# chongkuiqi/S2ANet

Measured on AMD Instinct MI355X. Metric: 1024x1024 DOTA chips/sec (R-50-FPN S2ANet inference), higher is better.
Workload: dtype f16; 1 GPU; BASELINE configs[2]: full R-50-FPN S2ANet inference, batch 8 of 1024x1024 synthetic uint8 chips per GPU; 3 independent batches in flight on 3 HIP streams; global_batch=8, num_classes=15, weights=seeded random init of the reference architecture; odm_cls bias calibrated, nms_candidate_cap=160000, nms_candidates_dropped=0, distinct_input_batches=3, fam_cls_branch=True, hip_graph=False, batches_in_flight=3, parallelism=dp1 (one process per GPU)

## Files before the change

include/s2anet_hip.h:

```cpp
#ifndef S2ANET_HIP_H_
#define S2ANET_HIP_H_

#include <stddef.h>
#include <stdint.h>

#ifdef __cplusplus
extern "C" {
#endif

#define S2A_OK 0
#define S2A_EINVAL (-1)
#define S2A_EWORKSPACE (-2)
#define S2A_EHIP (-3)
#define S2A_ENOTIMPL (-4)

#define S2A_DTYPE_F32 0
#define S2A_DTYPE_F16 1
#define S2A_DTYPE_F64 2

#define S2A_LAYOUT_NCHW 0
#define S2A_LAYOUT_NHWC 1

typedef void* s2a_stream_t;

// ... 217 lines not shown
int s2a_deform_conv_backward_input_f32(const float* input, const float* offset, const float* grad_output, const float* weight,
                                       float* grad_input, float* grad_offset, int64_t batch, int64_t channels,
                                       int64_t height, int64_t width, int64_t out_channels, void* workspace,
                                       size_t workspace_bytes, s2a_stream_t stream);

size_t s2a_deform_conv_backward_weight_workspace_bytes(int64_t batch, int64_t channels, int64_t height, int64_t width,
                                                       int64_t out_channels);
int s2a_deform_conv_backward_weight_f16(const void* input, const void* offset, const void* grad_output,
                                        float* grad_weight_f32, int64_t batch, int64_t channels, int64_t height,
                                        int64_t width, int64_t out_channels, void* workspace, size_t workspace_bytes,
                                        s2a_stream_t stream);

size_t s2a_deform_conv_backward_weight_f32_workspace_bytes(int64_t batch, int64_t channels, int64_t height, int64_t width,
                                                           int64_t out_channels);
int s2a_deform_conv_backward_weight_f32(const float* input, const float* offset, const float* grad_output,
                                        float* grad_weight, float scale, int64_t batch, int64_t channels, int64_t height,
                                        int64_t width, int64_t out_channels, void* workspace, size_t workspace_bytes,
                                        s2a_stream_t stream);

size_t s2a_deform_conv_backward_workspace_bytes(int dtype, int64_t batch, int64_t channels, int64_t height, int64_t width,
                                                int64_t out_channels);
int s2a_deform_conv_backward(int dtype, const void* input, const void* offset, const void* grad_output, const void* weight,
                             float* grad_input_f32, void* grad_offset, float* grad_weight_f32, float scale, int64_t batch,
                             int64_t channels, int64_t height, int64_t width, int64_t out_channels, void* workspace,
                             size_t workspace_bytes, s2a_stream_t stream);
int s2a_deform_conv_backward_typed(int dtype, const void* input, const void* offset, const void* grad_output,
                                   const void* weight, void* grad_input, void* grad_offset, float* grad_weight_f32,
                                   float scale, int64_t batch, int64_t channels, int64_t height, int64_t width,
                                   int64_t out_channels, void* workspace, size_t workspace_bytes, s2a_stream_t stream);

int s2a_conv3x3_tail1x1_f16(const void* x, const void* weight_frag, const void* bias, const void* tail_weight_frag,
                            const void* tail_bias, const void* residual, void* out, const void* chain_weight_frag,
                            const void* chain_bias, void* chain_out, int64_t chain_channels, int64_t batch, int64_t channels,
                            int64_t mid_channels, int64_t out_channels, int64_t height, int64_t width,
                            s2a_stream_t stream);

int s2a_conv1x1_chain_f16(const void* x, const void* weight_frag, const void* bias, const void* residual, void* out,
                          const void* chain_weight_frag, const void* chain_bias, void* chain_out, int64_t chain_channels,
                          int64_t batch, int64_t channels, int64_t out_channels, int64_t height, int64_t width,
                          s2a_stream_t stream);

int s2a_conv1x1_add_up2_f16(const void* x, const void* weight_frag, const void* bias, const void* coarse,
                            void* out, int64_t batch, int64_t channels, int64_t height, int64_t width,
                            int64_t out_channels, s2a_stream_t stream);

int64_t s2a_pyramid_pixels(const s2a_pyramid* pyr, int64_t batch);
int s2a_conv3x3_pyramid_f16(const void* x, const void* weight_frag, const void* bias, const void* residual,
                            void* out, int64_t batch, int64_t channels, int64_t out_channels, int relu,
                            const s2a_pyramid* pyr, s2a_stream_t stream);
int s2a_conv3x3_head_pyramid_f16(const void* x, const void* weight_frag, const void* bias, void* out,
                                 const void* head_weight_frag, const void* head_bias, void* head_out,
                                 int64_t batch, int64_t channels, int64_t out_channels, int relu,
                                 const s2a_pyramid* pyr, s2a_stream_t stream);
int s2a_orconv_pool_pyramid_f16(const void* x, const void* weight_frag, const void* bias, void* out, void* pooled,
                                int64_t batch, int64_t channels, int64_t out_channels, const s2a_pyramid* pyr,
                                s2a_stream_t stream);
int64_t s2a_conv_wino_packed_elems(int64_t out_channels, int64_t channels);
int s2a_conv_wino_pack_weight_f16(const void* weight, int64_t out_channels, int64_t channels, void* packed,
                                  s2a_stream_t stream);
int s2a_conv3x3_wino_pyramid_f16(const void* x, const void* weight_wino, const void* bias, void* out, void* pooled,
                                 int64_t batch, int64_t channels, int64_t out_channels, int relu,
                                 const s2a_pyramid* pyr, s2a_stream_t stream);
int s2a_align_conv_pyramid_f16(const void* x, const float* anchors, const void* weight_packed, void* out,
                               int64_t batch, int64_t channels, int64_t out_channels, int relu,
                               const s2a_pyramid* pyr, s2a_stream_t stream);
int s2a_fam_refine_anchors_pyramid(const void* pred, int64_t row_stride, int64_t batch, const s2a_pyramid* pyr,
                                   float anchor_scale, float* refined, s2a_stream_t stream);

int64_t s2a_stem_packed_elems(void);
int s2a_stem_pack_weight_f16(const void* weight, void* packed, s2a_stream_t stream);
int s2a_stem_u8_f16(const void* image_u8, const void* weight_packed, const void* bias, void* out,
                    int64_t batch, int64_t height, int64_t width, float divisor, s2a_stream_t stream);

#define S2A_LOSS_MAX_LEVELS 8

typedef struct s2a_loss_map {
  const void* cls;
  const void* bbox;
  const float* anchors;
  float* grad_cls;
  float* grad_bbox;
  int64_t anchor_batch_stride;
  int32_t height, width;
  int32_t cls_dtype, bbox_dtype;
  float fpn_balance;
  int32_t reserved;
} s2a_loss_map;

typedef struct s2a_loss_params {
  int32_t batch, num_classes, n_levels, reserved;
  float fl_gamma, fl_alpha, smooth_l1_beta, reg_balance, odm_balance;
  s2a_loss_map map[2][S2A_LOSS_MAX_LEVELS];
} s2a_loss_params;

size_t s2a_s2anet_loss_workspace_bytes(int64_t batch, int64_t anchors_per_image);
int s2a_s2anet_loss_forward(const s2a_loss_params* params, const int64_t* assign_ids, const float* targets,
                            const int64_t* target_offsets, float* loss, float* items, float* norm, void* workspace,
                            size_t workspace_bytes, s2a_stream_t stream);

typedef struct s2a_loss_grad_map {
  const float* src;
  void* dst;
  int64_t numel;
  int32_t dtype;
  int32_t norm_index;
} s2a_loss_grad_map;
// ... 50 lines not shown
```

s2anet_amd/_lib.py:

```python
import ctypes
import os
import subprocess

import torch

_HERE = os.path.dirname(os.path.abspath(__file__))
LIB_PATH = os.environ.get("S2A_LIB_PATH") or os.path.join(_HERE, "libs2anet_hip.so")

OK, EINVAL, EWORKSPACE, EHIP, ENOTIMPL = 0, -1, -2, -3, -4
DTYPE_F32, DTYPE_F16, DTYPE_F64 = 0, 1, 2
LAYOUT_NCHW, LAYOUT_NHWC = 0, 1

c_i64, c_int, c_f32, c_sz, c_vp = (ctypes.c_int64, ctypes.c_int, ctypes.c_float, ctypes.c_size_t,
                                   ctypes.c_void_p)


class DcnParams(ctypes.Structure):
    _fields_ = [("batch", c_i64), ("channels", c_i64), ("height", c_i64), ("width", c_i64),
                ("out_channels", c_i64),
                ("kW", c_int), ("kH", c_int), ("dW", c_int), ("dH", c_int), ("padW", c_int),
                ("padH", c_int), ("dilationW", c_int), ("dilationH", c_int), ("group", c_int),
                ("deformable_group", c_int), ("dtype", c_int), ("offset_dtype", c_int),
                ("layout", c_int), ("relu", c_int)]

# ... 98 lines not shown
    "s2a_s2anet_loss_workspace_bytes": (c_sz, [c_i64, c_i64]),
    "s2a_s2anet_loss_forward": (c_int, [ctypes.POINTER(LossParams), c_vp, c_vp, c_vp, c_vp, c_vp, c_vp, c_vp, c_sz, c_vp]),
    "s2a_s2anet_loss_backward": (c_int, [ctypes.POINTER(LossGradMap), c_int, c_vp, c_vp, c_vp]),
    "s2a_deform_conv_workspace_bytes": (c_sz, [ctypes.POINTER(DcnParams)]),
    "s2a_deform_conv_forward": (c_int, [c_vp, c_vp, c_vp, c_vp, ctypes.POINTER(DcnParams), c_vp,
                                        c_sz, c_vp]),
    "s2a_align_offsets": (c_int, [c_vp, c_i64, c_i64, c_i64, c_f32, c_int, c_vp, c_vp]),
    "s2a_align_conv_workspace_bytes": (c_sz, [ctypes.POINTER(AlignParams)]),
    "s2a_align_conv_forward": (c_int, [c_vp, c_vp, c_vp, c_vp, ctypes.POINTER(AlignParams), c_vp,
                                       c_sz, c_vp]),
    "s2a_dcn_packed_elems": (c_i64, [c_i64, c_i64, c_int]),
    "s2a_nms_small_stats": (c_int, [ctypes.POINTER(ctypes.c_int64), ctypes.POINTER(ctypes.c_int64)]),
    "s2a_dcn_pack_weight": (c_int, [c_vp, c_i64, c_i64, c_int, c_vp, c_vp]),
    "s2a_bias_act_nhwc": (c_int, [c_vp, c_vp, c_vp, c_i64, c_i64, c_int, c_int, c_vp]),
    "s2a_bias_act_nhwc_to": (c_int, [c_vp, c_vp, c_vp, c_vp, c_i64, c_i64, c_int, c_int, c_vp]),
    "s2a_conv_pack_weight_f16": (c_int, [c_vp, c_i64, c_i64, c_int, c_vp, c_vp]),
    "s2a_conv_nhwc_f16": (c_int, [c_vp, c_vp, c_vp, c_vp, c_vp, c_i64, c_i64, c_i64, c_i64, c_i64, c_int, c_int,
                                  c_int, c_vp]),
    "s2a_conv_pack_weight_train": (c_int, [c_vp, c_int, c_i64, c_i64, c_int, c_vp, c_vp, c_vp]),
    "s2a_conv_backward_prep_f16_workspace_bytes": (c_sz, [c_i64, c_i64]),
    "s2a_conv_backward_prep_f16": (c_int, [c_vp, c_vp, c_vp, c_vp, c_int, c_i64, c_i64, c_vp, c_sz, c_vp]),
    "s2a_conv_backward_weight_f16_workspace_bytes": (c_sz, [c_i64, c_i64, c_i64, c_i64, c_i64, c_int]),
    "s2a_conv_backward_weight_f16": (c_int, [c_vp, c_vp, c_vp, c_int, c_i64, c_i64, c_i64, c_i64, c_i64, c_int, c_vp, c_sz,
                                             c_vp]),
    "s2a_debug_read_stamps": (c_int, [c_vp, c_i64]),
    "s2a_build_flags": (c_int, []),
    "s2a_deform_conv_backward_input_workspace_bytes": (c_sz, [c_i64, c_i64, c_i64, c_i64, c_i64]),
    "s2a_deform_conv_backward_weight_workspace_bytes": (c_sz, [c_i64, c_i64, c_i64, c_i64, c_i64]),
    "s2a_deform_conv_backward_workspace_bytes": (c_sz, [c_int, c_i64, c_i64, c_i64, c_i64, c_i64]),
    "s2a_deform_conv_backward": (c_int, [c_int, c_vp, c_vp, c_vp, c_vp, c_vp, c_vp, c_vp, c_f32, c_i64, c_i64, c_i64, c_i64,
                                         c_i64, c_vp, c_sz, c_vp]),
    "s2a_deform_conv_backward_typed": (c_int, [c_int, c_vp, c_vp, c_vp, c_vp, c_vp, c_vp, c_vp, c_f32, c_i64, c_i64, c_i64, c_i64,
                                               c_i64, c_vp, c_sz, c_vp]),
    "s2a_deform_conv_backward_input_f32_workspace_bytes": (c_sz, [c_i64, c_i64, c_i64, c_i64, c_i64]),
    "s2a_deform_conv_backward_weight_f32_workspace_bytes": (c_sz, [c_i64, c_i64, c_i64, c_i64, c_i64]),
    "s2a_deform_conv_backward_weight_f32": (c_int, [c_vp, c_vp, c_vp, c_vp, c_f32, c_i64, c_i64, c_i64, c_i64, c_i64,
                                                    c_vp, c_sz, c_vp]),
    "s2a_deform_conv_backward_input_f32": (c_int, [c_vp, c_vp, c_vp, c_vp, c_vp, c_vp, c_i64, c_i64, c_i64, c_i64, c_i64,
                                                   c_vp, c_sz, c_vp]),
    "s2a_deform_conv_backward_weight_f16": (c_int, [c_vp, c_vp, c_vp, c_vp, c_i64, c_i64, c_i64, c_i64, c_i64, c_vp, c_sz, c_vp]),
    "s2a_deform_conv_backward_input_f16": (c_int, [c_vp, c_vp, c_vp, c_vp, c_vp, c_vp, c_i64, c_i64, c_i64, c_i64, c_i64,
                                           c_vp, c_sz, c_vp]),
    "s2a_deformable_im2col": (c_int, [c_vp, c_vp, c_vp, ctypes.POINTER(DcnParams), c_vp]),
    "s2a_deformable_col2im": (c_int, [c_vp, c_vp, c_vp, ctypes.POINTER(DcnParams), c_vp]),
    "s2a_deformable_col2im_coord": (c_int, [c_vp, c_vp, c_vp, c_vp, ctypes.POINTER(DcnParams), c_vp]),
    "s2a_conv3x3_tail1x1_f16": (c_int, [c_vp] * 10 + [c_i64] * 7 + [c_vp]),
    "s2a_conv1x1_chain_f16": (c_int, [c_vp] * 8 + [c_i64] * 6 + [c_vp]),
    "s2a_conv1x1_add_up2_f16": (c_int, [c_vp, c_vp, c_vp, c_vp, c_vp, c_i64, c_i64, c_i64, c_i64, c_i64, c_vp]),
    "s2a_pyramid_pixels": (c_i64, [ctypes.POINTER(Pyramid), c_i64]),
    "s2a_conv3x3_pyramid_f16": (c_int, [c_vp, c_vp, c_vp, c_vp, c_vp, c_i64, c_i64, c_i64, c_int,
                                        ctypes.POINTER(Pyramid), c_vp]),
    "s2a_conv3x3_head_pyramid_f16": (c_int, [c_vp, c_vp, c_vp, c_vp, c_vp, c_vp, c_vp, c_i64, c_i64, c_i64, c_int,
                                             ctypes.POINTER(Pyramid), c_vp]),
    "s2a_orconv_pool_pyramid_f16": (c_int, [c_vp, c_vp, c_vp, c_vp, c_vp, c_i64, c_i64, c_i64, ctypes.POINTER(Pyramid), c_vp]),
    "s2a_conv_wino_packed_elems": (c_i64, [c_i64, c_i64]),
    "s2a_conv_wino_pack_weight_f16": (c_int, [c_vp, c_i64, c_i64, c_vp, c_vp]),
    "s2a_conv3x3_wino_pyramid_f16": (c_int, [c_vp, c_vp, c_vp, c_vp, c_vp, c_i64, c_i64, c_i64, c_int,
                                             ctypes.POINTER(Pyramid), c_vp]),
    "s2a_align_conv_pyramid_f16": (c_int, [c_vp, c_vp, c_vp, c_vp, c_i64, c_i64, c_i64, c_int,
                                           ctypes.POINTER(Pyramid), c_vp]),
    "s2a_fam_refine_anchors_pyramid": (c_int, [c_vp, c_i64, c_i64, ctypes.POINTER(Pyramid), c_f32, c_vp, c_vp]),
    "s2a_stem_packed_elems": (c_i64, []),
    "s2a_stem_pack_weight_f16": (c_int, [c_vp, c_vp, c_vp]),
    "s2a_stem_u8_f16": (c_int, [c_vp, c_vp, c_vp, c_vp, c_i64, c_i64, c_i64, c_f32, c_vp]),
    "s2a_pyramid_candidates_count": (c_i64, [ctypes.POINTER(Pyramid), c_i64]),
    "s2a_pyramid_candidates": (c_int, [c_vp, c_vp, c_vp, c_i64, ctypes.POINTER(Pyramid), c_int, c_i64, c_f32, c_vp, c_vp, c_vp, c_vp]),
    "s2a_rbox_to_poly": (c_int, [c_vp, c_i64, c_i64, c_vp, c_vp]),
    "s2a_scene_gather_u8": (c_int, [c_vp, c_i64, c_i64, c_vp, c_i64, ctypes.c_int32, c_vp, c_vp]),
    "s2a_scene_merge_workspace_bytes": (c_sz, [c_i64, c_i64]),
    "s2a_scene_merge": (c_int, [c_vp, c_vp, c_vp, c_vp, c_vp, c_i64, c_i64, ctypes.c_int32, ctypes.c_double, c_i64,
                                c_vp, c_vp, c_vp, c_vp, c_vp, c_vp, c_vp, c_sz, c_vp]),
    "s2a_eval_task1_workspace_bytes": (c_sz, [c_i64, c_i64, ctypes.c_int32, ctypes.c_int32]),
    "s2a_eval_task1": (c_int, [c_vp, c_vp, c_vp, c_vp, c_i64, c_vp, c_vp, c_vp, c_vp, c_i64, ctypes.c_int32, ctypes.c_int32,
                               ctypes.c_double, c_int, c_int, ctypes.POINTER(ctypes.c_double)] + [c_vp] * 9 +
                       [ctypes.POINTER(EvalCurves), c_vp, c_sz, c_vp]),
    "s2a_train_update_workspace_bytes": (c_sz, [c_i64]),
    "s2a_train_update": (c_int, [ctypes.POINTER(TrainUpdateArgs), c_vp, c_sz, c_vp]),
    "s2a_delta2bbox_rotated": (c_int, [c_vp, c_vp, c_i64, c_f32, c_vp, c_vp]),
    "s2a_fam_refine_anchors": (c_int, [c_vp, c_i64, c_i64, c_i64, c_f32, c_f32, c_int, c_int,
                                       c_vp, c_vp]),
}


def build(force=False):
    csrc = os.path.join(_HERE, "csrc")
    if force:
        subprocess.check_call(["make", "-C", csrc, "-s", "clean"])
    subprocess.check_call(["make", "-C", csrc, "-s", "-j4"])
    return LIB_PATH


_lib = None


def lib():
    global _lib
    if _lib is None:
        if not os.path.exists(LIB_PATH):
            raise RuntimeError(
                f"{LIB_PATH} is missing: build it with `python -c 'import __graft_entry__ as g; "
                f"g.build()'` or `make -C s2anet_amd/csrc` — s2anet_amd has no CPU fallback")
        L = ctypes.CDLL(LIB_PATH)
        for name, (res, args) in SYMBOLS.items():
            fn = getattr(L, name)
            fn.restype, fn.argtypes = res, args
        flags = L.s2a_build_flags()
# ... 52 lines not shown
```

s2anet_amd/csrc/conv_ops.hip:

```cpp
#include <hip/hip_fp16.h>
#include <hip/hip_runtime.h>

#include <algorithm>
#include <cstdlib>
#include <type_traits>

#include "common.hpp"
#include "mfma_common.hpp"

namespace s2a {
namespace {

__global__ void k_pack_weight_frag(const _Float16* __restrict__ w, int O, int C, _Float16* __restrict__ wp,
                                   int taps = 9) {
  int64_t e = (int64_t)blockIdx.x * blockDim.x + threadIdx.x;
  int64_t total = (int64_t)O * C * taps;
  if (e >= total) return;
  const int G = O / 64;
  int j = (int)(e & 7);
  int lane = (int)((e >> 3) & 63);
  int kk = (int)((e >> 9) & 3);
  int mt = (int)((e >> 11) & 1);
  int64_t r = e >> 12;
  int g = (int)(r % G);
// ... 816 lines not shown
#pragma unroll
      for (int c4 = 0; c4 < 4; c4++)
#pragma unroll
        for (int kk = 0; kk < 4; kk++)
#pragma unroll
          for (int j = 0; j < 2; j++) {
            const V bf = *reinterpret_cast<const V*>(s_st + (32 * j + (lane & 31)) * kStRowB + (c4 * 64 + kk * 16 + (lane >> 5) * 8) * 2);
            c2[j] = __builtin_amdgcn_mfma_f32_32x32x16_f16(aw[c4 * 4 + kk], bf, c2[j], 0, 0, 0);
          }
    }
  }
  __syncthreads();
  constexpr int rowb = O3 * 2 + 16;
  if constexpr (C16) {
#pragma unroll
    for (int n = 0; n < NG3; n++)
#pragma unroll
      for (int a = 0; a < 4; a++) {
        const int och = (wave + 4 * n) * 64 + 16 * a + 4 * kg16;
        const h4e bq = *reinterpret_cast<const h4e*>(chain_b + och);
#pragma unroll
        for (int b = 0; b < 4; b++) {
          h2e lo = {(_Float16)(cacc[n][a][b][0] + (float)bq[0]), (_Float16)(cacc[n][a][b][1] + (float)bq[1])};
          h2e hi = {(_Float16)(cacc[n][a][b][2] + (float)bq[2]), (_Float16)(cacc[n][a][b][3] + (float)bq[3])};
          lo = __builtin_elementwise_max(lo, h2e{(_Float16)0.f, (_Float16)0.f});
          hi = __builtin_elementwise_max(hi, h2e{(_Float16)0.f, (_Float16)0.f});
          *reinterpret_cast<h4e*>(smem + (16 * b + pix16) * rowb + och * 2) = h4e{lo[0], lo[1], hi[0], hi[1]};
        }
      }
  } else {
#pragma unroll
    for (int j = 0; j < 2; j++)
#pragma unroll
      for (int rq = 0; rq < 4; rq++) {
        const int och = wave * 32 + 8 * rq + 4 * (lane >> 5);
        const h4e bq = *reinterpret_cast<const h4e*>(chain_b + och);
        h2e lo = {(_Float16)(c2[j][rq * 4] + (float)bq[0]), (_Float16)(c2[j][rq * 4 + 1] + (float)bq[1])};
        h2e hi = {(_Float16)(c2[j][rq * 4 + 2] + (float)bq[2]), (_Float16)(c2[j][rq * 4 + 3] + (float)bq[3])};
        lo = __builtin_elementwise_max(lo, h2e{(_Float16)0.f, (_Float16)0.f});
        hi = __builtin_elementwise_max(hi, h2e{(_Float16)0.f, (_Float16)0.f});
        *reinterpret_cast<h4e*>(smem + (32 * j + (lane & 31)) * rowb + och * 2) = h4e{lo[0], lo[1], hi[0], hi[1]};
      }
  }
  __syncthreads();
  constexpr int vpr = O3 / 8;
#pragma unroll
  for (int i = 0; i < kPos * vpr / 256; i++) {
    const int idx = tid + 256 * i, pos = idx / vpr, col = idx % vpr;
    if (g0 + pos < Ntot)
      *reinterpret_cast<V*>(chain_out + (g0 + pos) * O3 + col * 8) = *reinterpret_cast<const V*>(smem + pos * rowb + col * 16);
  }
}

}
}

using namespace s2a;

namespace s2a {
namespace {
template <int TAPS, int OG, int PH = 1, int SD = 1, bool TAIL = false, int HT = 0>
int launch_conv(const _Float16* x, const _Float16* wfrag, const _Float16* bias, const _Float16* residual,
                _Float16* out, int64_t B, int C, int H, int W, int Ho, int Wo, int cstride, int O, int relu,
                hipStream_t st, const LevelTab* levels = nullptr, int64_t level_tiles = 0, int res_up = 0,
                ConvExtra ex = ConvExtra{nullptr, nullptr, nullptr, nullptr, 1}) {
  using Cfg = ConvCfg<TAPS, OG, PH, SD, TAIL, HT>;
  const int64_t Ntot = B * (int64_t)Ho * Wo;
  int64_t tiles = TAPS == 9 ? B * ((Wo + 15) / 16) * ((Ho + Cfg::kTH - 1) / Cfg::kTH) : (Ntot + Cfg::kPos - 1) / Cfg::kPos;
  LevelTab lt = {};
  if (levels) { lt = *levels; tiles = level_tiles; }
  dim3 grid((unsigned)tiles, (unsigned)((O + 64 * OG - 1) / (64 * OG)));
  auto kern = k_conv_f16<TAPS, OG, PH, SD, TAIL, HT>;
  S2A_HIP(hipFuncSetAttribute(reinterpret_cast<const void*>(kern), hipFuncAttributeMaxDynamicSharedMemorySize, Cfg::kLds + Cfg::kBiasBytes));
  kern<<<grid, 256 * PH, Cfg::kLds + Cfg::kBiasBytes, st>>>(x, wfrag, bias, residual, out, Ntot, C, H, W, Ho, Wo, cstride, O, relu,
                                     (unsigned)((uint64_t)B * H * W * C * 2), lt, res_up, ex);
  S2A_LAUNCH_CHECK();
  return S2A_OK;
}

struct ConvCall {
  const _Float16 *x, *wfrag, *bias, *residual;
  _Float16* out;
  int64_t B;
  int C, H, W, Ho, Wo, cstride, O, relu;
  hipStream_t st;
  const LevelTab* levels = nullptr;
  int64_t level_tiles = 0;
  int res_up = 0;
  ConvExtra ex = ConvExtra{nullptr, nullptr, nullptr, nullptr, 1};
  template <int TAPS, int OG, int PH = 1, int SD = 1, bool TAIL = false, int HT = 0>
  int run() const {
    return launch_conv<TAPS, OG, PH, SD, TAIL, HT>(x, wfrag, bias, residual, out, B, C, H, W, Ho, Wo, cstride, O, relu, st, levels,
                                                   level_tiles, res_up, ex);
  }
};
}
}

extern "C" int s2a_conv_nhwc_f16(const void* x, const void* weight_frag, const void* bias, const void* residual,
                                 void* out, int64_t batch, int64_t channels, int64_t height, int64_t width,
                                 int64_t out_channels, int ksize, int stride, int relu, s2a_stream_t stream) {
  S2A_CHECK_ARG(batch >= 0 && channels > 0 && out_channels > 0 && height > 0 && width > 0, "conv: bad shape");
  S2A_CHECK_ARG(ksize == 3 || ksize == 1, "conv: kernel size must be 1 or 3");
  S2A_CHECK_ARG(stride == 1 || stride == 2, "conv: stride must be 1 or 2");
  S2A_CHECK_ARG(!(ksize == 3 && stride == 2) || out_channels % 128 == 0, "conv: 3x3 stride 2 needs out_channels % 128 == 0");
  S2A_CHECK_ARG((channels % 64 == 0 || channels == 32) && out_channels % 64 == 0,
// ... 184 lines not shown
  return conv3x3_pyramid_impl(x, weight_frag, bias, residual, out, ConvExtra{nullptr, nullptr, nullptr, nullptr, 1}, batch,
                              channels, out_channels, relu, pyr, stream);
}

extern "C" int s2a_conv3x3_head_pyramid_f16(const void* x, const void* weight_frag, const void* bias, void* out,
                                            const void* head_weight_frag, const void* head_bias, void* head_out,
                                            int64_t batch, int64_t channels, int64_t out_channels, int relu,
                                            const s2a_pyramid* pyr, s2a_stream_t stream) {
  S2A_CHECK_ARG(out_channels == 256, "conv3x3_head_pyramid: the fused 1x1 head needs a 256-channel tower");
  S2A_CHECK_ARG(head_weight_frag && head_bias && head_out, "conv3x3_head_pyramid: NULL head tensor");
  S2A_CHECK_ARG(((uintptr_t)head_weight_frag % 16) == 0 && ((uintptr_t)head_bias % 8) == 0 && ((uintptr_t)head_out % 16) == 0,
                "conv3x3_head_pyramid: misaligned head tensor");
  ConvExtra ex{nullptr, (const _Float16*)head_weight_frag, (const _Float16*)head_bias, (_Float16*)head_out, out != nullptr};
  return conv3x3_pyramid_impl(x, weight_frag, bias, nullptr, out ? out : head_out, ex, batch, channels, out_channels, relu,
                              pyr, stream);
}

extern "C" int s2a_orconv_pool_pyramid_f16(const void* x, const void* weight_frag, const void* bias, void* out,
                                           void* pooled, int64_t batch, int64_t channels, int64_t out_channels,
                                           const s2a_pyramid* pyr, s2a_stream_t stream) {
  S2A_CHECK_ARG(pooled != nullptr && ((uintptr_t)pooled % 16) == 0 && out_channels % 64 == 0,
                "orconv_pool_pyramid: pooled must be a 16-byte aligned buffer, out_channels a multiple of 64");
  return conv3x3_pyramid_impl(x, weight_frag, bias, nullptr, out, ConvExtra{(_Float16*)pooled, nullptr, nullptr, nullptr, 1},
                              batch, channels, out_channels, 0, pyr, stream);
}

static int conv3x3_pyramid_impl(const void* x, const void* weight_frag, const void* bias, const void* residual,
                                void* out, ConvExtra ex, int64_t batch, int64_t channels, int64_t out_channels,
                                int relu, const s2a_pyramid* pyr, s2a_stream_t stream) {
  S2A_CHECK_ARG(batch >= 0 && channels > 0 && out_channels > 0, "conv_pyramid: bad shape");
  S2A_CHECK_ARG((channels % 64 == 0 || channels == 32) && out_channels % 64 == 0,
                "conv_pyramid: channels must be 32 or a multiple of 64, out_channels a multiple of 64");
  LevelTab lt; int64_t pix = 0;
  int og = out_channels % 256 == 0 ? 4 : (out_channels % 128 == 0 ? 2 : 1);
  const char* og_env = getenv("S2A_CONV_OG");
  if (og_env && !ex.head_w) og = std::min(og, std::max(1, atoi(og_env)));
  int ph = (og == 4 && channels % 64 == 0) ? 2 : 1;
  if (const char* f = getenv("S2A_CONV_PH")) ph = atoi(f) == 2 && og == 4 && channels % 64 == 0 ? 2 : 1;
  const int64_t tiles = build_levels(pyr, batch, &lt, &pix, 8 * ph);
  S2A_CHECK_ARG(tiles >= 0, "conv_pyramid: bad level table (1..8 levels, positive sizes)");
  S2A_CHECK_ARG((uint64_t)pix * channels * 2 < (1ull << 31), "conv_pyramid: input too large for 32-bit offsets");
  if (batch == 0) return S2A_OK;
  S2A_CHECK_ARG(x && weight_frag && out, "conv_pyramid: NULL tensor");
  S2A_CHECK_ARG(((uintptr_t)x % 16) == 0 && ((uintptr_t)out % 16) == 0 && ((uintptr_t)weight_frag % 16) == 0 &&
                ((uintptr_t)bias % 8) == 0 && ((uintptr_t)residual % 16) == 0, "conv_pyramid: tensors must be 16-byte aligned");
  if (lt.n == 1) lt.n = 2, lt.tile0[1] = 0x7fffffff;
  hipStream_t st = as_stream(stream);
  const ConvCall c{(const _Float16*)x, (const _Float16*)weight_frag, (const _Float16*)bias, (const _Float16*)residual,
                   (_Float16*)out, batch, (int)channels, lt.H[0], lt.W[0], lt.H[0], lt.W[0], 1, (int)out_channels, relu, st,
                   &lt, tiles, 0, ex};
  if (ph == 2 && og == 4) return c.run<9, 4, 2>();
  return og == 4 ? c.run<9, 4>() : (og == 2 ? c.run<9, 2>() : c.run<9, 1>());
}
```

s2anet_amd/head.py:

```python
import math
import os

import numpy as np
import torch
import torch.nn as nn

from . import _lib
from .alignconv import AlignConv
from .loss import LOSS_DEFAULTS, grid_anchors, s2anet_loss
from .orn import ORConv2d, RotationInvariantPooling
from .rotated import assign_labels, assign_labels_batched, batched_multiclass_nms_rotated, multiclass_nms_rotated


def delta2bbox_rotated(rois, deltas, wh_ratio_clip=16 / 1000):
    _lib.require_cuda(rois, deltas)
    r, d = rois.float().contiguous(), deltas.float().contiguous()
    assert r.shape == d.shape and r.shape[-1] == 5
    out = torch.empty_like(r)
    n = r.numel() // 5
    with torch.cuda.device(r.device):
        _lib.check(_lib.lib().s2a_delta2bbox_rotated(_lib.ptr(r), _lib.ptr(d), n, float(wh_ratio_clip),
                                                     _lib.ptr(out), _lib.stream_ptr(r.device)))
    return out

# ... 100 lines not shown
                self.feat_channels % 64 == 0 and self.align_conv.kernel_size == (3, 3))

    def forward_pyramid(self, layout, x, anchors=None, trace=None):
        from . import pyramid as P

        wino = P.wino_enabled()

        def tower(seq, t):
            for blk in seq:
                if wino and blk[0].wino_ok() and blk[0].in_channels >= 128:
                    w, b, o = blk[0].packed_args_wino()
                    t = P.conv3x3_wino(layout, t, w, b, o, relu=True)
                    continue
                w, b, o = blk[0].packed_args()
                t = P.conv3x3(layout, t, w, b, o, relu=True)
            return t

        def tower_with_head(seq, head, t):
            fusable = (head.kernel_size == (1, 1) and head.out_channels <= 32 and seq[-1][0].out_channels == 256 and
                       seq[-1][0].in_channels % 64 == 0 and not os.environ.get("S2A_NO_FUSED_HEAD"))
            if not fusable:
                w, b, o = head.packed_args()
                return P.conv1x1(tower(seq, t), w, b, o, relu=False)
            t = tower(seq[:-1], t)
            w, b, o = seq[-1][0].packed_args()
            hw, hb, _ = head.packed_args()
            return P.conv3x3_head(layout, t, w, b, o, hw, hb, relu=True)

        fam_bbox = tower_with_head(self.fam_reg_ls, self.fam_reg_head, x)
        fam_cls = None
        if self.compute_fam_cls:
            fam_cls = tower_with_head(self.fam_cls_ls, self.fam_cls_head, x)
        own_anchors = P.fam_refine_anchors(layout, fam_bbox, self.anchor_scale)
        if anchors is None:
            anchors = own_anchors
        else:
            assert anchors.shape == own_anchors.shape and anchors.dtype == torch.float32 and anchors.is_contiguous()
        if getattr(self, "capture", None) is not None:
            self.capture.update(layout=layout, x=x, anchors=anchors)
        al = P.align_conv(layout, x, anchors, self.align_conv.packed_weight(torch.float16), self.feat_channels)
        wa = self.or_conv.rotate_arf()
        orc = self.or_conv.packed_cache()
        if self.or_pool.nOrientation == 8 and wa.shape[0] % 64 == 0 and wino and wa.shape[1] % 32 == 0:
            or_feat, pooled = P.conv3x3_wino(layout, al, orc.get_wino(wa),
                                             orc.get_bias(self.or_conv.bias, wa.shape[0]), wa.shape[0],
                                             relu=False, pool=True)
        elif self.or_pool.nOrientation == 8 and wa.shape[0] % 64 == 0:
            or_feat, pooled = P.orconv_pool(layout, al, orc.get(wa),
                                            orc.get_bias(self.or_conv.bias, wa.shape[0]), wa.shape[0])
        else:
            or_feat = P.conv3x3(layout, al, orc.get(wa),
                                orc.get_bias(self.or_conv.bias, wa.shape[0]), wa.shape[0], relu=False)
            pooled = P.rot_inv_pool(or_feat, self.or_pool.nOrientation)
        w, b, o = self.odm_cls_head.packed_args()
        odm_cls = P.conv3x3(layout, tower(self.odm_cls_ls, pooled), w, b, o, relu=False)
        w, b, o = self.odm_reg_head.packed_args()
        odm_bbox = P.conv3x3(layout, tower(self.odm_reg_ls, or_feat), w, b, o, relu=False)
        n = len(layout.sizes)
        if trace is not None:
            trace.update(x=x, fam_bbox=fam_bbox, fam_cls=fam_cls, own_anchors=own_anchors, anchors=anchors, align=al,
                         or_feat=or_feat, pooled=pooled, odm_cls=odm_cls, odm_bbox=odm_bbox)
        return PyramidPred(layout, odm_cls, odm_bbox, anchors,
                           [layout.level(fam_cls, l, self.num_classes) for l in range(n)] if fam_cls is not None else [None] * n,
                [layout.level(fam_bbox, l, 5) for l in range(n)],
                [layout.level(odm_cls, l, self.num_classes) for l in range(n)],
                [layout.level(odm_bbox, l, 5) for l in range(n)],
                [layout.rows(anchors, l).view(layout.batch, *layout.sizes[l], 5) for l in range(n)])

    def forward(self, feats, targets=None, imgs_size=None, post_process=False):
        if isinstance(targets, bool):
            targets, post_process = None, targets
        per_level = [self.forward_single(f, s) for f, s in zip(feats, self.featmap_strides)]
        p = tuple(map(list, zip(*per_level)))
        results = {"loss": None, "loss_items": None, "boxes_ls": None, "pred": None}
        if targets is not None:
            if imgs_size is None:
                raise ValueError("forward(feats, targets) needs imgs_size to scale the targets to pixels")
            self.imgs_size = tuple(int(v) for v in imgs_size)
            targets[:, [2, 4]] = targets[:, [2, 4]] * imgs_size[1]
            targets[:, [3, 5]] = targets[:, [3, 5]] * imgs_size[0]
            results["loss"], results["loss_items"] = self.compute_loss(p, targets)
        if post_process:
            results["boxes_ls"] = self.get_bboxes(p)
        if targets is None and not post_process:
            results["pred"] = p
        return results

    def init_grid_anchors(self, featmap_sizes, device):
        return [grid_anchors(hw, s, self.anchor_scale, device) for hw, s in zip(featmap_sizes, self.featmap_strides)]

    def _loss_pred(self, p):
        p = list(p)
        if len(p) == 5:
            sizes = [tuple(b.shape[2:]) for b in p[1]]
            p = p[:4] + [self.init_grid_anchors(sizes, p[1][0].device), p[4]]
        if len(p) != 6:
            raise ValueError(f"p must be the 5 per-level lists of forward() or the reference's 6, got {len(p)}")
        if any(t is None for t in p[0]):
            raise ValueError("compute_loss needs the FAM classification: this head was built with compute_fam_cls=False")
        return p

    def assign_labels_fam_odm(self, p, targets):
        p = self._loss_pred(p)
        B = p[1][0].shape[0]
        dev = p[1][0].device
        init_all = torch.cat([a.reshape(-1, 5) for a in p[4]], 0).float()
        refine_all = torch.cat([a.reshape(B, -1, 5) for a in p[5]], 1).detach().float()
        t = targets.detach().float().reshape(-1, 7)
        img = t[:, 0].long()
        order = torch.argsort(img, stable=True)
# ... 84 lines not shown
```

s2anet_amd/pyramid.py:

```python
import ctypes

import torch

from . import _lib


class PyramidLayout:

    def __init__(self, batch, sizes, strides):
        assert 1 <= len(sizes) <= 8 and len(sizes) == len(strides)
        self.batch, self.sizes, self.strides = int(batch), [tuple(map(int, s)) for s in sizes], list(strides)
        self.c = _lib.Pyramid()
        self.c.n_levels = len(sizes)
        self.pix0, p = [], 0
        for i, ((h, w), s) in enumerate(zip(self.sizes, strides)):
            self.c.height[i], self.c.width[i], self.c.stride[i] = h, w, float(s)
            self.pix0.append(p)
            p += self.batch * h * w
        self.pixels = p

    def key(self):
        return (self.batch, tuple(self.sizes), tuple(self.strides))

    def new(self, channels, device, dtype=torch.float16):
        return torch.empty((self.pixels, channels), dtype=dtype, device=device)

    def level(self, buf, l, channels=None):
        h, w = self.sizes[l]
        v = buf[self.pix0[l]:self.pix0[l] + self.batch * h * w].view(self.batch, h, w, buf.shape[1])
        if channels is not None:
            v = v[..., :channels]
        return v.permute(0, 3, 1, 2)

    def rows(self, buf, l):
        h, w = self.sizes[l]
        return buf[self.pix0[l]:self.pix0[l] + self.batch * h * w]


def conv3x3(layout, x, packed_w, bias, out_channels, relu, residual=None, out=None):
    L = _lib.lib()
    if out is None:
        out = layout.new(out_channels, x.device)
    with torch.cuda.device(x.device):
        _lib.check(L.s2a_conv3x3_pyramid_f16(_lib.ptr(x), _lib.ptr(packed_w), _lib.ptr(bias), _lib.ptr(residual),
                                             _lib.ptr(out), layout.batch, x.shape[1], out_channels, int(bool(relu)),
                                             ctypes.byref(layout.c), _lib.stream_ptr(x.device)))
    return out


def conv3x3_head(layout, x, packed_w, bias, out_channels, head_w, head_b, relu=True, keep_tower=False):
    L = _lib.lib()
    head_out = layout.new(64, x.device)
    tower = layout.new(out_channels, x.device) if keep_tower else None
    with torch.cuda.device(x.device):
        _lib.check(L.s2a_conv3x3_head_pyramid_f16(_lib.ptr(x), _lib.ptr(packed_w), _lib.ptr(bias), _lib.ptr(tower), _lib.ptr(head_w),
                                                  _lib.ptr(head_b), _lib.ptr(head_out), layout.batch, x.shape[1], out_channels,
                                                  int(bool(relu)), ctypes.byref(layout.c), _lib.stream_ptr(x.device)))
    return (head_out, tower) if keep_tower else head_out


def orconv_pool(layout, x, packed_w, bias, out_channels, n_orientation=8):
    assert n_orientation == 8
    L = _lib.lib()
    out = layout.new(out_channels, x.device)
    pooled = layout.new(out_channels // 8, x.device)
    with torch.cuda.device(x.device):
        _lib.check(L.s2a_orconv_pool_pyramid_f16(_lib.ptr(x), _lib.ptr(packed_w), _lib.ptr(bias), _lib.ptr(out), _lib.ptr(pooled),
                                                 layout.batch, x.shape[1], out_channels, ctypes.byref(layout.c),
                                                 _lib.stream_ptr(x.device)))
    return out, pooled


def conv3x3_wino(layout, x, packed_wino, bias, out_channels, relu, pool=False, out=None):
    L = _lib.lib()
    if out is None:
        out = layout.new(out_channels, x.device)
    pooled = layout.new(out_channels // 8, x.device) if pool else None
    with torch.cuda.device(x.device):
        _lib.check(L.s2a_conv3x3_wino_pyramid_f16(_lib.ptr(x), _lib.ptr(packed_wino), _lib.ptr(bias), _lib.ptr(out),
                                                  _lib.ptr(pooled), layout.batch, x.shape[1], out_channels, int(bool(relu)),
                                                  ctypes.byref(layout.c), _lib.stream_ptr(x.device)))
    return (out, pooled) if pool else out


def wino_enabled():
    import os
    return os.environ.get("S2A_CONV_WINO", "0") == "1"


def conv1x1(x, packed_w, bias, out_channels, relu, residual=None):
    L = _lib.lib()
    out = torch.empty((x.shape[0], out_channels), dtype=torch.float16, device=x.device)
    with torch.cuda.device(x.device):
# ... 49 lines not shown
```

Baseline: 2009 chips/s.

## Add narrow 16-output 3x3 conv kernel for ODM cls/reg heads

Adds a dedicated persistent 3x3 pyramid conv kernel for heads with at most 16 output maps (ODM cls with 15 classes and reg with 5). It computes only one 16-wide MFMA output group instead of a padded 64-channel group, keeps all weights resident in LDS, and triple-buffers input patches with buffer-load-to-LDS. The output is still written as 64-column rows with zero padding so downstream consumers are unchanged. The cost is a new hand-scheduled kernel with hardcoded wait counts, and a grid capped at 256 workgroups, which may underuse the GPU.

New measurement: 2035 chips/s (median of 6 runs). 1.01x the previous value.

```diff
diff --git a/include/s2anet_hip.h b/include/s2anet_hip.h
--- a/include/s2anet_hip.h
+++ b/include/s2anet_hip.h
@@ -293,6 +293,9 @@
                                  const void* head_weight_frag, const void* head_bias, void* head_out,
                                  int64_t batch, int64_t channels, int64_t out_channels, int relu,
                                  const s2a_pyramid* pyr, s2a_stream_t stream);
+int s2a_conv3x3_narrow_pyramid_f16(const void* x, const void* weight_frag, const void* bias, void* out, int64_t batch,
+                                   int64_t channels, int64_t out_channels_used, int relu, const s2a_pyramid* pyr,
+                                   s2a_stream_t stream);
 int s2a_orconv_pool_pyramid_f16(const void* x, const void* weight_frag, const void* bias, void* out, void* pooled,
                                 int64_t batch, int64_t channels, int64_t out_channels, const s2a_pyramid* pyr,
                                 s2a_stream_t stream);
diff --git a/s2anet_amd/_lib.py b/s2anet_amd/_lib.py
--- a/s2anet_amd/_lib.py
+++ b/s2anet_amd/_lib.py
@@ -174,6 +174,7 @@
                                         ctypes.POINTER(Pyramid), c_vp]),
     "s2a_conv3x3_head_pyramid_f16": (c_int, [c_vp, c_vp, c_vp, c_vp, c_vp, c_vp, c_vp, c_i64, c_i64, c_i64, c_int,
                                              ctypes.POINTER(Pyramid), c_vp]),
+    "s2a_conv3x3_narrow_pyramid_f16": (c_int, [c_vp, c_vp, c_vp, c_vp, c_i64, c_i64, c_i64, c_int, ctypes.POINTER(Pyramid), c_vp]),
     "s2a_orconv_pool_pyramid_f16": (c_int, [c_vp, c_vp, c_vp, c_vp, c_vp, c_i64, c_i64, c_i64, ctypes.POINTER(Pyramid), c_vp]),
     "s2a_conv_wino_packed_elems": (c_i64, [c_i64, c_i64]),
     "s2a_conv_wino_pack_weight_f16": (c_int, [c_vp, c_i64, c_i64, c_vp, c_vp]),
diff --git a/s2anet_amd/csrc/conv_ops.hip b/s2anet_amd/csrc/conv_ops.hip
--- a/s2anet_amd/csrc/conv_ops.hip
+++ b/s2anet_amd/csrc/conv_ops.hip
@@ -892,6 +892,184 @@
   }
 }
 
+constexpr int kNarrowPatch = ConvCfg<9, 1>::kPatchBytes;
+constexpr int kNarrowJ = ConvCfg<9, 1>::kJ;
+constexpr int kNarrowDma = ConvCfg<9, 1>::kDma;
+constexpr int kNarrowOutBytes = 128 * 32;
+constexpr int kNarrowFixedLds = 3 * kNarrowPatch + 2 * kNarrowOutBytes + 64;
+constexpr int kNarrowMaxC = 256;
+inline int narrow_lds_bytes(int C) { return kNarrowFixedLds + (C / 64) * 9 * 2048; }
+
+__global__ __launch_bounds__(256, 1) void k_conv3x3_narrow_f16(const _Float16* __restrict__ x,
+                                                               const _Float16* __restrict__ wfrag,
+                                                               const _Float16* __restrict__ bias,
+                                                               _Float16* __restrict__ out, int C, int O_used, int relu,
+                                                               unsigned x_bytes, LevelTab lt, int tiles) {
+  using T = _Float16;
+  using V = f16x8;
+  using h2e = __attribute__((ext_vector_type(2))) _Float16;
+  using h4e = __attribute__((ext_vector_type(4))) _Float16;
+  extern __shared__ __attribute__((aligned(16))) char smem[];
+  const int tid = threadIdx.x, lane = tid & 63, wave = tid >> 6;
+  const int wave_u = __builtin_amdgcn_readfirstlane(wave);
+  const int CC = C / 64, nstage = 9 * CC;
+  char* s_w = smem + 3 * kNarrowPatch;
+  char* s_out = s_w + nstage * 2048;
+  T* s_bias = reinterpret_cast<T*>(s_out + 2 * kNarrowOutBytes);
+  const int t_begin = (int)((int64_t)blockIdx.x * tiles / gridDim.x);
+  const int t_end = (int)((int64_t)(blockIdx.x + 1) * tiles / gridDim.x);
+  if (t_begin >= t_end) return;
+  const unsigned row_bytes = (unsigned)C * 2;
+  const __amdgpu_buffer_rsrc_t rx = __builtin_amdgcn_make_buffer_rsrc(const_cast<T*>(x), 0, (int)x_bytes, 0x00020000);
+
+  struct Tile { int H, W, ty0, tx0; int64_t base; };
+  auto decode = [&](int tile) {
+    int t0 = 0, p0 = 0, H = lt.H[0], W = lt.W[0];
+#pragma unroll
+    for (int i = 1; i < kMaxLevels; i++)
+      if (i < lt.n && tile >= lt.tile0[i]) {
+        t0 = lt.tile0[i]; p0 = lt.pix0[i]; H = lt.H[i]; W = lt.W[i];
+      }
+    const int txn = (W + 15) / 16, tyn = (H + 7) / 8, loc = tile - t0;
+    const int bimg = loc / (txn * tyn), trem = loc % (txn * tyn);
+    return Tile{H, W, (trem / txn) * 8, (trem % txn) * 16, (int64_t)p0 + (int64_t)bimg * H * W};
+  };
+  unsigned pvoff[kNarrowJ];
+  auto bind = [&](const Tile& tl) {
+#pragma unroll
+    for (int j = 0; j < kNarrowJ; j++) {
+      const int v = (wave_u + 4 * j) * 64 + lane, p = v / 9, q = v % 9;
+      const int yy = tl.ty0 - 1 + p / kCPW, xx = tl.tx0 - 1 + p % kCPW;
+      const bool in = q < 8 && p < ConvCfg<9, 1>::kPix && yy >= 0 && yy < tl.H && xx >= 0 && xx < tl.W;
+      pvoff[j] = in ? (unsigned)((tl.base + (int64_t)yy * tl.W + xx) * row_bytes + q * 16) : 0x80000000u;
+    }
+  };
+  auto piece_issue = [&](int buf, int cc, int j) {
+    const int i = wave_u + 4 * j;
+    if (i < kNarrowDma)
+      __builtin_amdgcn_raw_ptr_buffer_load_lds(rx, (__attribute__((address_space(3))) void*)(smem + buf * kNarrowPatch + i * 1024),
+                                               16, (int)pvoff[j], cc * 128, 0, 0);
+  };
+  auto patch_issue = [&](int buf, int cc) {
+#pragma unroll
+    for (int j = 0; j < kNarrowJ; j++) piece_issue(buf, cc, j);
+  };
+
+  int itile = t_begin, icc = 0;
+  bool ivalid = true;
+  auto advance = [&]() {
+    if (++icc == CC) {
+      icc = 0;
+      if (++itile < t_end) bind(decode(itile)); else ivalid = false;
+    }
+  };
+  bind(decode(t_begin));
+  patch_issue(0, 0);
+  advance();
+  if (ivalid) {
+    patch_issue(1, icc);
+    advance();
+  }
+  for (int idx = tid; idx < nstage * 128; idx += 256) {
+    const int s = idx >> 7, ks = (idx >> 6) & 1, l = idx & 63;
+    *reinterpret_cast<V*>(s_w + idx * 16) =
+        reinterpret_cast<const V*>(wfrag)[(int64_t)s * 512 + ks * 64 + ((l >> 4) & 1) * 128 + (l >> 5) * 32 + (l & 15)];
+  }
+  if (tid < 16) s_bias[tid] = (bias && tid < O_used) ? bias[tid] : (T)0.f;
+
+  const int kg16 = lane >> 4, i16 = lane & 15;
+  const int pix16 = (i16 >= 4 && i16 < 12) ? (((i16 - 4) >> 1) * 4 + (i16 & 1))
+                                           : (((i16 & 3) >> 1) * 4 + 2 + (i16 & 1) + (i16 >= 12 ? 8 : 0));
+  const int fbase16 = (2 * wave * kCPW + pix16) * kRowBytes + (kg16 & 1) * 64 + (kg16 >> 1) * 16;
+  constexpr int kTile16 = kCPW * kRowBytes;
+  const bool relu_u = __builtin_amdgcn_readfirstlane(relu) != 0;
+  f32x4 acc[2];
+#pragma unroll
+  for (int b = 0; b < 2; b++)
+#pragma unroll
+    for (int r = 0; r < 4; r++) acc[b][r] = 0.f;
+  __syncthreads();
+
+  auto stage_sync = [&](bool issued) {
+    __builtin_amdgcn_sched_barrier(0);
+    if (!issued) asm volatile("s_waitcnt vmcnt(0) lgkmcnt(0)\n\ts_barrier" ::: "memory");
+    else if (wave_u + 4 * (kNarrowJ - 1) < kNarrowDma) asm volatile("s_waitcnt vmcnt(7) lgkmcnt(0)\n\ts_barrier" ::: "memory");
+    else asm volatile("s_waitcnt vmcnt(6) lgkmcnt(0)\n\ts_barrier" ::: "memory");
+    __builtin_amdgcn_sched_barrier(0);
+  };
+  static_assert(kNarrowJ == 7 && kNarrowDma == 26, "stage_sync counts 7 pieces on waves 0-1 and 6 on waves 2-3");
+  int rb = 0;
+  for (int tile = t_begin; tile < t_end; tile++) {
+    const Tile cur = decode(tile);
+    bool issued = false;
+    for (int cc = 0; cc < CC; cc++) {
+      const bool more = ivalid;
+      issued = more;
+      const int ncc = icc, wb = rb == 0 ? 2 : rb - 1, buf = rb;
+      const char* P = smem + buf * kNarrowPatch + fbase16;
+      const char* Wc = s_w + cc * (9 * 2048) + lane * 16;
+      V fa[3][2], fp[3][2][2];
+      auto load_tap = [&](int t, V (&a)[2], V (&p)[2][2]) {
+        const int toff = ((t / 3) * kCPW + (t % 3)) * kRowBytes;
+#pragma unroll
+        for (int ks = 0; ks < 2; ks++) {
+          a[ks] = *reinterpret_cast<const V*>(Wc + (t * 2 + ks) * 1024);
+          p[ks][0] = *reinterpret_cast<const V*>(P + toff + ks * 32);
+          p[ks][1] = *reinterpret_cast<const V*>(P + kTile16 + toff + ks * 32);
+        }
+      };
+      load_tap(0, fa[0], fp[0]);
+      load_tap(1, fa[1], fp[1]);
+#pragma unroll
+      for (int t = 0; t < 9; t++) {
+        if (t + 2 < 9) load_tap(t + 2, fa[(t + 2) % 3], fp[(t + 2) % 3]);
+        if (t < kNarrowJ && more) piece_issue(wb, ncc, t);
+#pragma unroll
+        for (int ks = 0; ks < 2; ks++) {
+          acc[0] = __builtin_amdgcn_mfma_f32_16x16x32_f16(fa[t % 3][ks], fp[t % 3][ks][0], acc[0], 0, 0, 0);
+          acc[1] = __builtin_amdgcn_mfma_f32_16x16x32_f16(fa[t % 3][ks], fp[t % 3][ks][1], acc[1], 0, 0, 0);
+        }
+        __builtin_amdgcn_sched_barrier(0);
+      }
+      if (more) advance();
+      rb = rb == 2 ? 0 : rb + 1;
+      if (cc + 1 < CC) stage_sync(more);
+    }
+    char* so = s_out + ((tile - t_begin) & 1) * kNarrowOutBytes;
+    {
+      const int och = 4 * kg16;
+      const h4e bq = *reinterpret_cast<const h4e*>(s_bias + och);
+#pragma unroll
+      for (int b = 0; b < 2; b++) {
+        h2e lo = {(_Float16)(acc[b][0] + (float)bq[0]), (_Float16)(acc[b][1] + (float)bq[1])};
+        h2e hi = {(_Float16)(acc[b][2] + (float)bq[2]), (_Float16)(acc[b][3] + (float)bq[3])};
+        if (relu_u) {
+          lo = __builtin_elementwise_max(lo, h2e{(_Float16)0.f, (_Float16)0.f});
+          hi = __builtin_elementwise_max(hi, h2e{(_Float16)0.f, (_Float16)0.f});
+        }
+        h4e v4 = {lo[0], lo[1], hi[0], hi[1]};
+#pragma unroll
+        for (int e = 0; e < 4; e++)
+          if (och + e >= O_used) v4[e] = (_Float16)0.f;
+        *reinterpret_cast<h4e*>(so + (16 * (2 * wave + b) + pix16) * 32 + och * 2) = v4;
+#pragma unroll
+        for (int r = 0; r < 4; r++) acc[b][r] = 0.f;
+      }
+    }
+    stage_sync(issued);
+#pragma unroll
+    for (int i = 0; i < 4; i++) {
+      const int idx = tid + 256 * i, pos = idx >> 3, col = idx & 7;
+      const int y = cur.ty0 + (pos >> 4), xq = cur.tx0 + (pos & 15);
+      V v;
+#pragma unroll
+      for (int e = 0; e < 8; e++) v[e] = (_Float16)0.f;
+      if (col < 2) v = *reinterpret_cast<const V*>(so + pos * 32 + col * 16);
+      if (y < cur.H && xq < cur.W) *reinterpret_cast<V*>(out + (cur.base + (int64_t)y * cur.W + xq) * 64 + col * 8) = v;
+    }
+  }
+}
+
 }
 }
 
@@ -1182,3 +1360,35 @@
   if (ph == 2 && og == 4) return c.run<9, 4, 2>();
   return og == 4 ? c.run<9, 4>() : (og == 2 ? c.run<9, 2>() : c.run<9, 1>());
 }
+
+extern "C" int s2a_conv3x3_narrow_pyramid_f16(const void* x, const void* weight_frag, const void* bias, void* out,
+                                              int64_t batch, int64_t channels, int64_t out_channels_used, int relu,
+                                              const s2a_pyramid* pyr, s2a_stream_t stream) {
+  S2A_CHECK_ARG(batch >= 0 && channels > 0, "conv_narrow_pyramid: bad shape");
+  S2A_CHECK_ARG(channels % 64 == 0, "conv_narrow_pyramid: channels must be a multiple of 64");
+  S2A_CHECK_ARG(out_channels_used >= 1 && out_channels_used <= 16, "conv_narrow_pyramid: 1..16 maps (out_channels_used)");
+  bool narrow = channels <= kNarrowMaxC;
+  if (const char* f = getenv("S2A_CONV_NARROW")) narrow = narrow && atoi(f) != 0;
+  if (!narrow)
+    return conv3x3_pyramid_impl(x, weight_frag, bias, nullptr, out, ConvExtra{nullptr, nullptr, nullptr, nullptr, 1}, batch,
+                                channels, 64, relu, pyr, stream);
+  LevelTab lt; int64_t pix = 0;
+  const int64_t tiles = build_levels(pyr, batch, &lt, &pix, 8);
+  S2A_CHECK_ARG(tiles >= 0, "conv_narrow_pyramid: bad level table (1..8 levels, positive sizes)");
+  S2A_CHECK_ARG((uint64_t)pix * channels * 2 < (1ull << 31), "conv_narrow_pyramid: input too large for 32-bit offsets");
+  if (batch == 0) return S2A_OK;
+  S2A_CHECK_ARG(x && weight_frag && out, "conv_narrow_pyramid: NULL tensor");
+  S2A_CHECK_ARG(((uintptr_t)x % 16) == 0 && ((uintptr_t)out % 16) == 0 && ((uintptr_t)weight_frag % 16) == 0 &&
+                ((uintptr_t)bias % 8) == 0, "conv_narrow_pyramid: tensors must be 16-byte aligned");
+  int64_t grid = std::min<int64_t>(tiles, 256);
+  if (const char* f = getenv("S2A_CONV_NARROW_WGS")) grid = std::min<int64_t>(grid, std::max(1, atoi(f)));
+  const int lds = narrow_lds_bytes((int)channels);
+  auto kern = k_conv3x3_narrow_f16;
+  S2A_HIP(hipFuncSetAttribute(reinterpret_cast<const void*>(kern), hipFuncAttributeMaxDynamicSharedMemorySize, lds));
+  kern<<<dim3((unsigned)grid), 256, lds, as_stream(stream)>>>((const _Float16*)x, (const _Float16*)weight_frag,
+                                                               (const _Float16*)bias, (_Float16*)out, (int)channels,
+                                                               (int)out_channels_used, relu,
+                                                               (unsigned)((uint64_t)pix * channels * 2), lt, (int)tiles);
+  S2A_LAUNCH_CHECK();
+  return S2A_OK;
+}
diff --git a/s2anet_amd/head.py b/s2anet_amd/head.py
--- a/s2anet_amd/head.py
+++ b/s2anet_amd/head.py
@@ -176,10 +176,10 @@
             or_feat = P.conv3x3(layout, al, orc.get(wa),
                                 orc.get_bias(self.or_conv.bias, wa.shape[0]), wa.shape[0], relu=False)
             pooled = P.rot_inv_pool(or_feat, self.or_pool.nOrientation)
-        w, b, o = self.odm_cls_head.packed_args()
-        odm_cls = P.conv3x3(layout, tower(self.odm_cls_ls, pooled), w, b, o, relu=False)
-        w, b, o = self.odm_reg_head.packed_args()
-        odm_bbox = P.conv3x3(layout, tower(self.odm_reg_ls, or_feat), w, b, o, relu=False)
+        w, b, _ = self.odm_cls_head.packed_args()
+        odm_cls = P.conv3x3(layout, tower(self.odm_cls_ls, pooled), w, b, self.odm_cls_head.out_channels, relu=False)
+        w, b, _ = self.odm_reg_head.packed_args()
+        odm_bbox = P.conv3x3(layout, tower(self.odm_reg_ls, or_feat), w, b, self.odm_reg_head.out_channels, relu=False)
         n = len(layout.sizes)
         if trace is not None:
             trace.update(x=x, fam_bbox=fam_bbox, fam_cls=fam_cls, own_anchors=own_anchors, anchors=anchors, align=al,
diff --git a/s2anet_amd/pyramid.py b/s2anet_amd/pyramid.py
--- a/s2anet_amd/pyramid.py
+++ b/s2anet_amd/pyramid.py
@@ -39,6 +39,16 @@
 
 def conv3x3(layout, x, packed_w, bias, out_channels, relu, residual=None, out=None):
     L = _lib.lib()
+    if out_channels <= 16 and residual is None and x.shape[1] % 64 == 0:
+        if out is None:
+            out = layout.new(64, x.device)
+        assert out.shape == (layout.pixels, 64) and out.is_contiguous(), "the 16-row kernel stores rows of 64 columns"
+        with torch.cuda.device(x.device):
+            _lib.check(L.s2a_conv3x3_narrow_pyramid_f16(_lib.ptr(x), _lib.ptr(packed_w), _lib.ptr(bias), _lib.ptr(out),
+                                                        layout.batch, x.shape[1], out_channels, int(bool(relu)),
+                                                        ctypes.byref(layout.c), _lib.stream_ptr(x.device)))
+        return out
+    out_channels = max(64, out_channels)
     if out is None:
         out = layout.new(out_channels, x.device)
     with torch.cuda.device(x.device):
```
